# mhamilton723/STEGO

Measured on NVIDIA H100. Metric: train-step images/sec, higher is better.
Workload: dtype bf16

## Files before the change

profiles/attn_bench.py:

```python
import argparse
import os
import sys

import torch

sys.path.insert(0, os.path.dirname(os.path.dirname(os.path.abspath(__file__))))
from stego_b200 import _lib, ops
from _measure import call_ms, card, emit

CHECKS = [(1, 128, 1, 1.5), (2, 785, 6, 1.5), (1, 1601, 12, 1.5), (3, 50, 6, 1.5), (1, 257, 2, 1.5), (1, 3137, 2, 1.0),
          (2, 65, 6, 3.0), (1, 129, 1, 1.0), (1, 256, 3, 1.0), (2, 400, 2, 4.0), (1, 17, 1, 1.0)]


def ref(qkv, B, N, heads):
    E = heads * 64
    q, k, v = qkv.float().view(B, N, 3, heads, 64).permute(2, 0, 3, 1, 4)
    attn = ((q @ k.transpose(-2, -1)) * 0.125).softmax(-1)
    return (attn @ v).transpose(1, 2).reshape(B * N, E)


def rel(a, b):
    return ((a.double() - b.double()).norm() / b.double().norm()).item()


def main():
    ap = argparse.ArgumentParser()
    ap.add_argument("--check-only", action="store_true", help="run the correctness checks only")
    args = ap.parse_args()
    if os.environ.get("STEGO_PROFILE_LIB"):
        _lib.LIB_PATH = os.path.abspath(os.environ["STEGO_PROFILE_LIB"])
    dev = torch.device("cuda:0")
    res = dict(card=card(), check=[])
    torch.manual_seed(3)
    ok = True
    for B, N, heads, scale in CHECKS:
        E = heads * 64
        qkv = (torch.randn(B * N, 3 * E, device=dev) * scale).bfloat16()
        out = torch.full((B * N, E), float("nan"), device=dev, dtype=torch.bfloat16)
        ops.attention(qkv, out, B, N, E, heads)
        torch.cuda.synchronize()
        e = rel(out, ref(qkv, B, N, heads))
        fin = bool(torch.isfinite(out.float()).all())
        res["check"].append(dict(B=B, N=N, heads=heads, scale=scale, rel_l2=e, finite=fin))
        ok &= fin and e < 1e-2
    res["check_ok"] = ok
    if ok and not args.check_only:
        res["time"] = []
        flush = torch.zeros(64 * 1024 * 1024, device=dev)
        for name, B, N, heads in [("c1", 64, 785, 6), ("c2", 64, 1601, 12), ("c3", 32, 3137, 12)]:
            E = heads * 64
            qkv = torch.randn(B * N, 3 * E, device=dev).bfloat16()
            out = torch.empty(B * N, E, device=dev, dtype=torch.bfloat16)
            for _ in range(3):
                ops.attention(qkv, out, B, N, E, heads)
            torch.cuda.synchronize()
            tot = 0.0
            iters = 10
            for _ in range(iters):
                flush.add_(1.0)
                tot += call_ms(lambda: ops.attention(qkv, out, B, N, E, heads))[0]
            ms = tot / iters
            fl = 4.0 * B * heads * N * N * 64
            res["time"].append(dict(config=name, B=B, N=N, heads=heads, us=round(ms * 1e3, 1),
                                    tflops=round(fl / ms / 1e9)))
    emit(res)
    sys.exit(0 if ok else 1)


if __name__ == "__main__":
    main()
```

stego_b200/csrc/attention.cu:

```cuda
#include <stdlib.h>

#include "common.cuh"
#include "host_util.h"

namespace stego {

constexpr int ATT_BQ = 128;
constexpr int ATT_BKV = 64;
constexpr int ATT_D = 64;
constexpr int ATT_STAGES = 4;
constexpr int ATT_THREADS = 288;

constexpr uint32_t ATT_Q_BYTES = 128 * 64 * 2;
constexpr uint32_t ATT_KV_BYTES = 64 * 64 * 2;
constexpr uint32_t ATT_SMEM_Q = 0;
constexpr uint32_t ATT_SMEM_KV = ATT_Q_BYTES;
constexpr uint32_t ATT_SMEM_BAR = ATT_SMEM_KV + ATT_STAGES * 2 * ATT_KV_BYTES;
constexpr uint32_t ATT_SMEM_TOTAL = ATT_SMEM_BAR + 128;

struct AttnParams {
  int N;
  int E;
  float scale_log2e;
};

__global__ void __launch_bounds__(ATT_THREADS, 2)
attention_fwd_kernel(const __grid_constant__ CUtensorMap tmQKV, const __grid_constant__ CUtensorMap tmOut, AttnParams p) {
  extern __shared__ __align__(1024) uint8_t smem[];
  if ((smem_u32(smem) & 1023u) != 0u) __trap();
  uint64_t* bars = reinterpret_cast<uint64_t*>(smem + ATT_SMEM_BAR);
  uint64_t* q_full = bars;
  uint64_t* kv_full = bars + 1;
  uint64_t* kv_empty = kv_full + ATT_STAGES;

  const int warp = threadIdx.x >> 5;
  const int lane = threadIdx.x & 31;
  const int q0 = blockIdx.x * ATT_BQ;
  const int head = blockIdx.y;
  const int img = blockIdx.z;
  const int nkv = (p.N + ATT_BKV - 1) / ATT_BKV;

  if (threadIdx.x == 0) {
    mbar_init(q_full, 1);
    for (int s = 0; s < ATT_STAGES; ++s) {
      mbar_init(&kv_full[s], 1);
      mbar_init(&kv_empty[s], 2);
    }
    fence_barrier_init();
  }
  __syncthreads();

  if (warp == 8) {
    if (lane == 0) {
      tma_prefetch_desc(&tmQKV);
      tma_prefetch_desc(&tmOut);
      mbar_arrive_expect_tx(q_full, ATT_Q_BYTES);
      tma_load_3d(smem + ATT_SMEM_Q, &tmQKV, q_full, head * ATT_D, q0, img);
      tma_load_3d(smem + ATT_SMEM_Q + ATT_Q_BYTES / 2, &tmQKV, q_full, head * ATT_D, q0 + 64, img);
      uint32_t stage = 0, phase = 0;
      for (int j = 0; j < nkv; ++j) {
        mbar_wait(&kv_empty[stage], phase ^ 1u);
        uint8_t* sk = smem + ATT_SMEM_KV + stage * 2 * ATT_KV_BYTES;
        mbar_arrive_expect_tx(&kv_full[stage], 2 * ATT_KV_BYTES);
        tma_load_3d(sk, &tmQKV, &kv_full[stage], p.E + head * ATT_D, j * ATT_BKV, img);
        tma_load_3d(sk + ATT_KV_BYTES, &tmQKV, &kv_full[stage], 2 * p.E + head * ATT_D, j * ATT_BKV, img);
        if (++stage == ATT_STAGES) { stage = 0; phase ^= 1u; }
      }
    }
    return;
  }

  const int wg = warp >> 2;
  const int wq = warp & 3;
  const bool leader = (threadIdx.x & 127) == 0;
  const float c = p.scale_log2e;
  constexpr uint32_t DESC_HI = smem_desc_hi_sw128(1024);
  uint8_t* sq = smem + ATT_SMEM_Q + wg * (ATT_Q_BYTES / 2);
  const uint32_t q_lo = smem_desc_lo(smem_u32(sq), 16);
  const uint32_t k_lo0 = smem_desc_lo(smem_u32(smem + ATT_SMEM_KV), 16);
  const uint32_t v_lo0 = smem_desc_lo(smem_u32(smem + ATT_SMEM_KV + ATT_KV_BYTES), 8192);
  float o[32];
#pragma unroll
  for (int i = 0; i < 32; ++i) o[i] = 0.f;
  float m_run[2] = {-INFINITY, -INFINITY}, l_run[2] = {0.f, 0.f};
  mbar_wait(q_full, 0);
  uint32_t stage = 0, phase = 0;
  for (int j = 0; j < nkv; ++j) {
    mbar_wait(&kv_full[stage], phase);
    const uint32_t k_lo = k_lo0 + stage * ((2 * ATT_KV_BYTES) >> 4);
    const uint32_t v_lo = v_lo0 + stage * ((2 * ATT_KV_BYTES) >> 4);
    float s[32];
    wgmma_fence();
#pragma unroll
    for (uint32_t k = 0; k < ATT_D / 16; ++k)
      wgmma_ss<64, 0, 0>(s, smem_desc_join(q_lo + k * 2, DESC_HI), smem_desc_join(k_lo + k * 2, DESC_HI), k > 0 ? 1u : 0u);
    wgmma_commit();
    wgmma_wait<0>();
    fence_operands(s);
    const int valid = p.N - j * ATT_BKV;
    if (valid < ATT_BKV) {
#pragma unroll
      for (int i = 0; i < 32; ++i)
        if (8 * (i >> 2) + 2 * (lane & 3) + (i & 1) >= valid) s[i] = -INFINITY;
    }
    float alpha[2], mc[2];
#pragma unroll
    for (int h = 0; h < 2; ++h) {
      float mx = -INFINITY;
#pragma unroll
      for (int i = 0; i < 8; ++i) mx = fmaxf(mx, fmaxf(s[4 * i + 2 * h], s[4 * i + 2 * h + 1]));
      mx = fmaxf(mx, __shfl_xor_sync(0xffffffffu, mx, 1));
      mx = fmaxf(mx, __shfl_xor_sync(0xffffffffu, mx, 2));
      const float m_new = fmaxf(m_run[h], mx);
      alpha[h] = ex2_approx((m_run[h] - m_new) * c);
      m_run[h] = m_new;
      mc[h] = m_new * c;
    }
    uint32_t a[4][4];
    float rs[2] = {0.f, 0.f};
#pragma unroll
    for (int i = 0; i < 8; ++i) {
#pragma unroll
      for (int h = 0; h < 2; ++h) {
        const float e0 = ex2_approx(fmaf(s[4 * i + 2 * h], c, -mc[h]));
        const float e1 = ex2_approx(fmaf(s[4 * i + 2 * h + 1], c, -mc[h]));
        rs[h] += e0 + e1;
        a[i >> 1][(i & 1) * 2 + h] = pack_bf16x2(e0, e1);
      }
    }
#pragma unroll
    for (int h = 0; h < 2; ++h) l_run[h] = l_run[h] * alpha[h] + rs[h];
#pragma unroll
    for (int i = 0; i < 32; ++i) o[i] *= alpha[(i >> 1) & 1];
    wgmma_fence();
#pragma unroll
    for (uint32_t kk = 0; kk < ATT_BKV / 16; ++kk)
      wgmma_rs_n64<1>(o, a[kk], smem_desc_join(v_lo + kk * (2048u >> 4), DESC_HI), 1u);
    wgmma_commit();
    wgmma_wait<0>();
    fence_operands(o);
    if (leader) mbar_arrive(&kv_empty[stage]);
    if (++stage == ATT_STAGES) { stage = 0; phase ^= 1u; }
  }
  float inv[2];
#pragma unroll
  for (int h = 0; h < 2; ++h) {
    float l = l_run[h];
    l += __shfl_xor_sync(0xffffffffu, l, 1);
    l += __shfl_xor_sync(0xffffffffu, l, 2);
    inv[h] = __fdividef(1.0f, l);
  }
#pragma unroll
  for (int i = 0; i < 8; ++i) {
#pragma unroll
    for (int h = 0; h < 2; ++h) {
      const uint32_t r = static_cast<uint32_t>(wq * 16 + (lane >> 2) + 8 * h);
      const uint32_t off = sw128_offset(r, static_cast<uint32_t>(i)) + 4u * static_cast<uint32_t>(lane & 3);
      *reinterpret_cast<uint32_t*>(sq + off) = pack_bf16x2(o[4 * i + 2 * h] * inv[h], o[4 * i + 2 * h + 1] * inv[h]);
    }
  }
  fence_proxy_async_smem();
  asm volatile("bar.sync %0, 128;\n" ::"r"(wg + 1) : "memory");
  if (leader) {
    tma_store_3d(sq, &tmOut, head * ATT_D, q0 + wg * 64, img);
    tma_commit_group();
    tma_wait_group_read<0>();
  }
}

constexpr int PRB_STAGES = 4;
constexpr int PRB_PITCH = 72;
constexpr uint32_t PRB_SMEM_K = ATT_Q_BYTES;
constexpr uint32_t PRB_SMEM_STAGE = PRB_SMEM_K + PRB_STAGES * ATT_KV_BYTES;
constexpr uint32_t PRB_WARP_STAGE_BYTES = 16 * PRB_PITCH * 4;
constexpr uint32_t PRB_SMEM_BAR = PRB_SMEM_STAGE + 8 * PRB_WARP_STAGE_BYTES;
constexpr uint32_t PRB_SMEM_TOTAL = PRB_SMEM_BAR + 128;

__device__ __forceinline__ void st_global_cs(float* p, float v) {
  asm volatile("st.global.cs.f32 [%0], %1;\n" ::"l"(p), "f"(v) : "memory");
}

__global__ void __launch_bounds__(ATT_THREADS, 2)
attention_probs_kernel(const __grid_constant__ CUtensorMap tmQKV, float* __restrict__ probs, AttnParams p) {
  extern __shared__ __align__(1024) uint8_t smem[];
  if ((smem_u32(smem) & 1023u) != 0u) __trap();
  uint64_t* bars = reinterpret_cast<uint64_t*>(smem + PRB_SMEM_BAR);
  uint64_t* q_full = bars;
  uint64_t* k_full = bars + 1;
  uint64_t* k_empty = k_full + PRB_STAGES;

  const int warp = threadIdx.x >> 5;
  const int lane = threadIdx.x & 31;
  const int q0 = blockIdx.x * ATT_BQ;
  const int head = blockIdx.y;
  const int img = blockIdx.z;
  const int nkv = (p.N + ATT_BKV - 1) / ATT_BKV;

  if (threadIdx.x == 0) {
    mbar_init(q_full, 1);
    for (int s = 0; s < PRB_STAGES; ++s) {
      mbar_init(&k_full[s], 1);
      mbar_init(&k_empty[s], 2);
    }
    fence_barrier_init();
  }
  __syncthreads();

  if (warp == 8) {
    if (lane == 0) {
      tma_prefetch_desc(&tmQKV);
      mbar_arrive_expect_tx(q_full, ATT_Q_BYTES);
      tma_load_3d(smem, &tmQKV, q_full, head * ATT_D, q0, img);
      tma_load_3d(smem + ATT_Q_BYTES / 2, &tmQKV, q_full, head * ATT_D, q0 + 64, img);
      uint32_t stage = 0, phase = 0;
      for (int j = 0; j < 2 * nkv; ++j) {
        mbar_wait(&k_empty[stage], phase ^ 1u);
        mbar_arrive_expect_tx(&k_full[stage], ATT_KV_BYTES);
        tma_load_3d(smem + PRB_SMEM_K + stage * ATT_KV_BYTES, &tmQKV, &k_full[stage], p.E + head * ATT_D,
                    (j < nkv ? j : j - nkv) * ATT_BKV, img);
        if (++stage == PRB_STAGES) { stage = 0; phase ^= 1u; }
      }
    }
    return;
  }

  const int wg = warp >> 2;
  const int wq = warp & 3;
  const bool leader = (threadIdx.x & 127) == 0;
  const float c = p.scale_log2e;
  constexpr uint32_t DESC_HI = smem_desc_hi_sw128(1024);
  const uint32_t q_lo = smem_desc_lo(smem_u32(smem + wg * (ATT_Q_BYTES / 2)), 16);
  const uint32_t k_lo0 = smem_desc_lo(smem_u32(smem + PRB_SMEM_K), 16);
  float* stage_tile = reinterpret_cast<float*>(smem + PRB_SMEM_STAGE + warp * PRB_WARP_STAGE_BYTES);
  const int row0 = q0 + wg * 64 + wq * 16;
  float m_run[2] = {-INFINITY, -INFINITY}, l_run[2] = {0.f, 0.f};
  float inv[2] = {0.f, 0.f};
  mbar_wait(q_full, 0);
  uint32_t stage = 0, phase = 0;
  for (int j = 0; j < 2 * nkv; ++j) {
    const bool store_pass = j >= nkv;
    const int kt = store_pass ? j - nkv : j;
    mbar_wait(&k_full[stage], phase);
    const uint32_t k_lo = k_lo0 + stage * (ATT_KV_BYTES >> 4);
    float s[32];
    wgmma_fence();
#pragma unroll
    for (uint32_t k = 0; k < ATT_D / 16; ++k)
      wgmma_ss<64, 0, 0>(s, smem_desc_join(q_lo + k * 2, DESC_HI), smem_desc_join(k_lo + k * 2, DESC_HI), k > 0 ? 1u : 0u);
    wgmma_commit();
    wgmma_wait<0>();
    fence_operands(s);
    if (leader) mbar_arrive(&k_empty[stage]);
    if (++stage == PRB_STAGES) { stage = 0; phase ^= 1u; }
    const int valid = p.N - kt * ATT_BKV;
    if (!store_pass) {
      if (valid < ATT_BKV) {
#pragma unroll
        for (int i = 0; i < 32; ++i)
          if (8 * (i >> 2) + 2 * (lane & 3) + (i & 1) >= valid) s[i] = -INFINITY;
      }
#pragma unroll
      for (int h = 0; h < 2; ++h) {
        float mx = -INFINITY;
#pragma unroll
        for (int i = 0; i < 8; ++i) mx = fmaxf(mx, fmaxf(s[4 * i + 2 * h], s[4 * i + 2 * h + 1]));
        mx = fmaxf(mx, __shfl_xor_sync(0xffffffffu, mx, 1));
        mx = fmaxf(mx, __shfl_xor_sync(0xffffffffu, mx, 2));
        const float m_new = fmaxf(m_run[h], mx);
        const float alpha = ex2_approx((m_run[h] - m_new) * c);
        float rs = 0.f;
#pragma unroll
        for (int i = 0; i < 8; ++i)
          rs += ex2_approx((s[4 * i + 2 * h] - m_new) * c) + ex2_approx((s[4 * i + 2 * h + 1] - m_new) * c);
        l_run[h] = l_run[h] * alpha + rs;
        m_run[h] = m_new;
      }
      if (kt == nkv - 1) {
#pragma unroll
        for (int h = 0; h < 2; ++h) {
          float l = l_run[h];
          l += __shfl_xor_sync(0xffffffffu, l, 1);
          l += __shfl_xor_sync(0xffffffffu, l, 2);
          inv[h] = __frcp_rn(l);
        }
      }
      continue;
    }
    __syncwarp();
#pragma unroll
    for (int i = 0; i < 8; ++i) {
#pragma unroll
      for (int h = 0; h < 2; ++h) {
        const float p0 = ex2_approx((s[4 * i + 2 * h] - m_run[h]) * c) * inv[h];
        const float p1 = ex2_approx((s[4 * i + 2 * h + 1] - m_run[h]) * c) * inv[h];
        float2* dst = reinterpret_cast<float2*>(stage_tile + ((lane >> 2) + 8 * h) * PRB_PITCH + 8 * i + 2 * (lane & 3));
        *dst = make_float2(p0, p1);
      }
    }
    __syncwarp();
    const int nrows = min(16, p.N - row0);
    const size_t plane = (static_cast<size_t>(img) * gridDim.y + head) * static_cast<size_t>(p.N);
    float* out = probs + (plane + static_cast<size_t>(row0)) * static_cast<size_t>(p.N) + static_cast<size_t>(kt) * ATT_BKV;
#pragma unroll 4
    for (int r = 0; r < nrows; ++r) {
      float* orow = out + static_cast<size_t>(r) * static_cast<size_t>(p.N);
      if (lane < valid) st_global_cs(orow + lane, stage_tile[r * PRB_PITCH + lane]);
      if (lane + 32 < valid) st_global_cs(orow + lane + 32, stage_tile[r * PRB_PITCH + lane + 32]);
    }
  }
}

}

using namespace stego;

extern "C" int stego_attention_fwd(const void* qkv, void* out, int B, int N, int E, int heads, void* stream_) {
  cudaStream_t stream = reinterpret_cast<cudaStream_t>(stream_);
  STEGO_CHECK_ARG(qkv && out, "stego_attention_fwd: null pointer");
  STEGO_CHECK_ARG(B > 0 && N > 0 && heads > 0, "stego_attention_fwd: bad sizes");
  STEGO_CHECK_ARG(E == heads * ATT_D, "stego_attention_fwd: head_dim must be 64 (E=%d heads=%d)", E, heads);
  STEGO_CHECK_ARG((reinterpret_cast<uintptr_t>(out) & 15u) == 0, "stego_attention_fwd: out not 16-byte aligned");
  CUtensorMap tm;
  uint64_t dims[3] = {(uint64_t)3 * E, (uint64_t)N, (uint64_t)B};
  uint64_t str[2] = {(uint64_t)3 * E * 2, (uint64_t)N * 3 * E * 2};
  uint32_t box[3] = {64, 64, 1};
  int rc = make_tmap_bf16(&tm, qkv, 3, dims, str, box);
  if (rc != STEGO_OK) return rc;
  CUtensorMap tmo;
  uint64_t odims[3] = {(uint64_t)E, (uint64_t)N, (uint64_t)B};
  uint64_t ostr[2] = {(uint64_t)E * 2, (uint64_t)N * E * 2};
  if ((rc = make_tmap_bf16(&tmo, out, 3, odims, ostr, box)) != STEGO_OK) return rc;
  if ((rc = opt_in_smem<attention_fwd_kernel>(ATT_SMEM_TOTAL, "attention_fwd_kernel")) != STEGO_OK) return rc;
  AttnParams p;
  p.N = N;
  p.E = E;
  p.scale_log2e = 0.125f * 1.4426950408889634f;
  dim3 grid((N + ATT_BQ - 1) / ATT_BQ, heads, B);
  attention_fwd_kernel<<<grid, ATT_THREADS, ATT_SMEM_TOTAL, stream>>>(tm, tmo, p);
  STEGO_CHECK_LAUNCH("attention_fwd_kernel");
  return STEGO_OK;
}

extern "C" int stego_attention_probs(const void* qkv, float* probs, int B, int N, int E, int heads, void* stream_) {
  cudaStream_t stream = reinterpret_cast<cudaStream_t>(stream_);
  STEGO_CHECK_ARG(qkv && probs, "stego_attention_probs: null pointer");
  STEGO_CHECK_ARG(B > 0 && N > 0 && heads > 0, "stego_attention_probs: bad sizes");
  STEGO_CHECK_ARG(B <= 65535 && heads <= 65535, "stego_attention_probs: B and heads must be <= 65535");
  STEGO_CHECK_ARG(E == heads * ATT_D, "stego_attention_probs: head_dim must be 64 (E=%d heads=%d)", E, heads);
  STEGO_CHECK_ARG((reinterpret_cast<uintptr_t>(probs) & 3u) == 0, "stego_attention_probs: probs not 4-byte aligned");
  CUtensorMap tm;
  uint64_t dims[3] = {(uint64_t)3 * E, (uint64_t)N, (uint64_t)B};
  uint64_t str[2] = {(uint64_t)3 * E * 2, (uint64_t)N * 3 * E * 2};
  uint32_t box[3] = {64, 64, 1};
  int rc = make_tmap_bf16(&tm, qkv, 3, dims, str, box);
  if (rc != STEGO_OK) return rc;
  if ((rc = opt_in_smem<attention_probs_kernel>(PRB_SMEM_TOTAL, "attention_probs_kernel")) != STEGO_OK) return rc;
  AttnParams p;
  p.N = N;
  p.E = E;
  p.scale_log2e = 0.125f * 1.4426950408889634f;
  dim3 grid((N + ATT_BQ - 1) / ATT_BQ, heads, B);
  attention_probs_kernel<<<grid, ATT_THREADS, PRB_SMEM_TOTAL, stream>>>(tm, probs, p);
  STEGO_CHECK_LAUNCH("attention_probs_kernel");
  return STEGO_OK;
}
```

stego_b200/csrc/common.cuh:

```cuda
#pragma once
#include <cuda.h>
#include <cuda_bf16.h>
#include <cuda_runtime.h>
#include <stdint.h>
#include <stdio.h>

namespace stego {

typedef __nv_bfloat16 bf16;

__device__ __forceinline__ uint32_t smem_u32(const void* p) {
  return static_cast<uint32_t>(__cvta_generic_to_shared(p));
}
__device__ __forceinline__ uint32_t lane_id() { return threadIdx.x & 31u; }

__device__ __forceinline__ float warp_sum(float v) {
#pragma unroll
  for (int o = 16; o > 0; o >>= 1) v += __shfl_xor_sync(0xffffffffu, v, o);
  return v;
}
__device__ __forceinline__ float warp_max(float v) {
#pragma unroll
  for (int o = 16; o > 0; o >>= 1) v = fmaxf(v, __shfl_xor_sync(0xffffffffu, v, o));
  return v;
}

__device__ __forceinline__ void mbar_init(uint64_t* bar, uint32_t count) {
  asm volatile("mbarrier.init.shared::cta.b64 [%0], %1;\n" ::"r"(smem_u32(bar)), "r"(count) : "memory");
}
__device__ __forceinline__ void fence_barrier_init() {
  asm volatile("fence.mbarrier_init.release.cluster;\n" ::: "memory");
}
__device__ __forceinline__ void fence_proxy_async_smem() {
  asm volatile("fence.proxy.async.shared::cta;\n" ::: "memory");
}
__device__ __forceinline__ void mbar_arrive(uint64_t* bar) {
  asm volatile("mbarrier.arrive.shared::cta.b64 _, [%0];\n" ::"r"(smem_u32(bar)) : "memory");
}
__device__ __forceinline__ void mbar_arrive_expect_tx(uint64_t* bar, uint32_t bytes) {
  asm volatile("mbarrier.arrive.expect_tx.shared::cta.b64 _, [%0], %1;\n" ::"r"(smem_u32(bar)), "r"(bytes)
               : "memory");
}
__device__ __forceinline__ bool mbar_try_wait(uint64_t* bar, uint32_t parity) {
  uint32_t ok;
  asm volatile(
      "{\n\t.reg .pred P1;\n\t"
      "mbarrier.try_wait.parity.shared::cta.b64 P1, [%1], %2, %3;\n\t"
      "selp.b32 %0, 1, 0, P1;\n\t}\n"
      : "=r"(ok)
      : "r"(smem_u32(bar)), "r"(parity), "r"(1000000u)
      : "memory");
  return ok != 0;
}

__device__ __forceinline__ bool mbar_test_wait(uint64_t* bar, uint32_t parity) {
  uint32_t ok;
  asm volatile(
      "{\n\t.reg .pred P1;\n\t"
      "mbarrier.test_wait.parity.shared::cta.b64 P1, [%1], %2;\n\t"
      "selp.b32 %0, 1, 0, P1;\n\t}\n"
      : "=r"(ok)
      : "r"(smem_u32(bar)), "r"(parity)
      : "memory");
  return ok != 0;
}

#ifndef STEGO_MBAR_TIMEOUT_NS
#define STEGO_MBAR_TIMEOUT_NS 4000000000ull
#endif
__device__ __forceinline__ uint64_t globaltimer_ns() {
  uint64_t t;
  asm volatile("mov.u64 %0, %%globaltimer;\n" : "=l"(t));
  return t;
}
__device__ __forceinline__ void mbar_wait(uint64_t* bar, uint32_t parity) {
  if (mbar_test_wait(bar, parity)) return;
  if (mbar_try_wait(bar, parity)) return;
  uint32_t spins = 0;
  uint64_t t0 = 0;
  while (!mbar_try_wait(bar, parity)) {
    if ((++spins & 0x3Fu) == 0) {
      const uint64_t now = globaltimer_ns();
      if (t0 == 0) {
        t0 = now;
      } else if (now - t0 > STEGO_MBAR_TIMEOUT_NS) {
        __trap();
      }
    }
  }
}

__device__ __forceinline__ void tma_prefetch_desc(const CUtensorMap* m) {
  asm volatile("prefetch.tensormap [%0];\n" ::"l"(reinterpret_cast<uint64_t>(m)) : "memory");
}
__device__ __forceinline__ void tma_load_2d(void* smem_dst, const CUtensorMap* m, uint64_t* bar, int c0, int c1) {
  asm volatile(
      "cp.async.bulk.tensor.2d.shared::cluster.global.mbarrier::complete_tx::bytes [%0], [%1, {%3, %4}], [%2];\n" ::"r"(
          smem_u32(smem_dst)),
      "l"(reinterpret_cast<uint64_t>(m)), "r"(smem_u32(bar)), "r"(c0), "r"(c1)
      : "memory");
}
__device__ __forceinline__ void tma_load_3d(void* smem_dst, const CUtensorMap* m, uint64_t* bar, int c0, int c1,
                                            int c2) {
  asm volatile(
      "cp.async.bulk.tensor.3d.shared::cluster.global.mbarrier::complete_tx::bytes [%0], [%1, {%3, %4, %5}], "
      "[%2];\n" ::"r"(smem_u32(smem_dst)),
      "l"(reinterpret_cast<uint64_t>(m)), "r"(smem_u32(bar)), "r"(c0), "r"(c1), "r"(c2)
      : "memory");
}

__device__ __forceinline__ void tma_prefetch_l2_2d(const CUtensorMap* m, int c0, int c1) {
  asm volatile("cp.async.bulk.prefetch.tensor.2d.L2.global [%0, {%1, %2}];\n" ::"l"(reinterpret_cast<uint64_t>(m)),
               "r"(c0), "r"(c1)
               : "memory");
}

__device__ __forceinline__ void tma_store_3d(uint32_t smem_src, const CUtensorMap* m, int c0, int c1, int c2) {
  asm volatile("cp.async.bulk.tensor.3d.global.shared::cta.bulk_group [%0, {%2, %3, %4}], [%1];\n" ::"l"(
                   reinterpret_cast<uint64_t>(m)),
               "r"(smem_src), "r"(c0), "r"(c1), "r"(c2)
               : "memory");
}
__device__ __forceinline__ void tma_store_3d(const void* smem_src, const CUtensorMap* m, int c0, int c1, int c2) {
  tma_store_3d(smem_u32(smem_src), m, c0, c1, c2);
}
__device__ __forceinline__ void tma_reduce_add_3d(uint32_t smem_src, const CUtensorMap* m, int c0, int c1, int c2) {
  asm volatile("cp.reduce.async.bulk.tensor.3d.global.shared::cta.add.bulk_group [%0, {%2, %3, %4}], [%1];\n" ::"l"(
                   reinterpret_cast<uint64_t>(m)),
               "r"(smem_src), "r"(c0), "r"(c1), "r"(c2)
               : "memory");
}

__device__ __forceinline__ void st_shared_b32(uint32_t addr, uint32_t v) {
  asm volatile("st.shared.b32 [%0], %1;\n" ::"r"(addr), "r"(v) : "memory");
}
__device__ __forceinline__ void st_shared_v2_f32(uint32_t addr, float a, float b) {
  asm volatile("st.shared.v2.f32 [%0], {%1, %2};\n" ::"r"(addr), "f"(a), "f"(b) : "memory");
}
__device__ __forceinline__ void tma_commit_group() { asm volatile("cp.async.bulk.commit_group;\n" ::: "memory"); }
template <int kPending>
__device__ __forceinline__ void tma_wait_group_read() {
  asm volatile("cp.async.bulk.wait_group.read %0;\n" ::"n"(kPending) : "memory");
}
template <int kPending>
__device__ __forceinline__ void tma_wait_group() {
  asm volatile("cp.async.bulk.wait_group %0;\n" ::"n"(kPending) : "memory");
}

__device__ __forceinline__ void named_bar_sync(int id, int threads) {
  asm volatile("bar.sync %0, %1;\n" ::"r"(id), "r"(threads) : "memory");
}

__device__ __forceinline__ void wgmma_fence() { asm volatile("wgmma.fence.sync.aligned;\n" ::: "memory"); }
__device__ __forceinline__ void wgmma_commit() { asm volatile("wgmma.commit_group.sync.aligned;\n" ::: "memory"); }
template <int kPending>
__device__ __forceinline__ void wgmma_wait() {
  asm volatile("wgmma.wait_group.sync.aligned %0;\n" ::"n"(kPending) : "memory");
}
template <int kN>
__device__ __forceinline__ void fence_operands(float (&d)[kN]) {
#pragma unroll
  for (int i = 0; i < kN; ++i) asm volatile("" : "+f"(d[i])::"memory");
}

template <int kTransA, int kTransB>
__device__ __forceinline__ void wgmma_ss_n64(float (&d)[32], uint64_t desc_a, uint64_t desc_b, uint32_t accumulate) {
  asm volatile(
      "{\n\t.reg .pred p;\n\tsetp.ne.b32 p, %34, 0;\n\t"
      "wgmma.mma_async.sync.aligned.m64n64k16.f32.bf16.bf16 {%0, %1, %2, %3, %4, %5, %6, %7, %8, %9, %10, %11, %12, %13, %14, %15, %16, %17, %18, %19, %20, %21, %22, %23, %24, %25, %26, %27, %28, %29, %30, %31}, %32, %33, p, 1, 1, %35, %36;\n\t}\n"
      : "+f"(d[0]), "+f"(d[1]), "+f"(d[2]), "+f"(d[3]), "+f"(d[4]), "+f"(d[5]), "+f"(d[6]), "+f"(d[7]), "+f"(d[8]), "+f"(d[9]), "+f"(d[10]), "+f"(d[11]), "+f"(d[12]), "+f"(d[13]), "+f"(d[14]), "+f"(d[15]), "+f"(d[16]), "+f"(d[17]), "+f"(d[18]), "+f"(d[19]), "+f"(d[20]), "+f"(d[21]), "+f"(d[22]), "+f"(d[23]), "+f"(d[24]), "+f"(d[25]), "+f"(d[26]), "+f"(d[27]), "+f"(d[28]), "+f"(d[29]), "+f"(d[30]), "+f"(d[31])
      : "l"(desc_a), "l"(desc_b), "r"(accumulate), "n"(kTransA), "n"(kTransB));
}

template <int kTransA, int kTransB>
__device__ __forceinline__ void wgmma_ss_n128(float (&d)[64], uint64_t desc_a, uint64_t desc_b, uint32_t accumulate) {
  asm volatile(
      "{\n\t.reg .pred p;\n\tsetp.ne.b32 p, %66, 0;\n\t"
      "wgmma.mma_async.sync.aligned.m64n128k16.f32.bf16.bf16 {%0, %1, %2, %3, %4, %5, %6, %7, %8, %9, %10, %11, %12, %13, %14, %15, %16, %17, %18, %19, %20, %21, %22, %23, %24, %25, %26, %27, %28, %29, %30, %31, %32, %33, %34, %35, %36, %37, %38, %39, %40, %41, %42, %43, %44, %45, %46, %47, %48, %49, %50, %51, %52, %53, %54, %55, %56, %57, %58, %59, %60, %61, %62, %63}, %64, %65, p, 1, 1, %67, %68;\n\t}\n"
      : "+f"(d[0]), "+f"(d[1]), "+f"(d[2]), "+f"(d[3]), "+f"(d[4]), "+f"(d[5]), "+f"(d[6]), "+f"(d[7]), "+f"(d[8]), "+f"(d[9]), "+f"(d[10]), "+f"(d[11]), "+f"(d[12]), "+f"(d[13]), "+f"(d[14]), "+f"(d[15]), "+f"(d[16]), "+f"(d[17]), "+f"(d[18]), "+f"(d[19]), "+f"(d[20]), "+f"(d[21]), "+f"(d[22]), "+f"(d[23]), "+f"(d[24]), "+f"(d[25]), "+f"(d[26]), "+f"(d[27]), "+f"(d[28]), "+f"(d[29]), "+f"(d[30]), "+f"(d[31]), "+f"(d[32]), "+f"(d[33]), "+f"(d[34]), "+f"(d[35]), "+f"(d[36]), "+f"(d[37]), "+f"(d[38]), "+f"(d[39]), "+f"(d[40]), "+f"(d[41]), "+f"(d[42]), "+f"(d[43]), "+f"(d[44]), "+f"(d[45]), "+f"(d[46]), "+f"(d[47]), "+f"(d[48]), "+f"(d[49]), "+f"(d[50]), "+f"(d[51]), "+f"(d[52]), "+f"(d[53]), "+f"(d[54]), "+f"(d[55]), "+f"(d[56]), "+f"(d[57]), "+f"(d[58]), "+f"(d[59]), "+f"(d[60]), "+f"(d[61]), "+f"(d[62]), "+f"(d[63])
      : "l"(desc_a), "l"(desc_b), "r"(accumulate), "n"(kTransA), "n"(kTransB));
}

template <int kTransA, int kTransB>
__device__ __forceinline__ void wgmma_ss_n256(float (&d)[128], uint64_t desc_a, uint64_t desc_b, uint32_t accumulate) {
  asm volatile(
      "{\n\t.reg .pred p;\n\tsetp.ne.b32 p, %130, 0;\n\t"
      "wgmma.mma_async.sync.aligned.m64n256k16.f32.bf16.bf16 {%0, %1, %2, %3, %4, %5, %6, %7, %8, %9, %10, %11, %12, %13, %14, %15, %16, %17, %18, %19, %20, %21, %22, %23, %24, %25, %26, %27, %28, %29, %30, %31, %32, %33, %34, %35, %36, %37, %38, %39, %40, %41, %42, %43, %44, %45, %46, %47, %48, %49, %50, %51, %52, %53, %54, %55, %56, %57, %58, %59, %60, %61, %62, %63, %64, %65, %66, %67, %68, %69, %70, %71, %72, %73, %74, %75, %76, %77, %78, %79, %80, %81, %82, %83, %84, %85, %86, %87, %88, %89, %90, %91, %92, %93, %94, %95, %96, %97, %98, %99, %100, %101, %102, %103, %104, %105, %106, %107, %108, %109, %110, %111, %112, %113, %114, %115, %116, %117, %118, %119, %120, %121, %122, %123, %124, %125, %126, %127}, %128, %129, p, 1, 1, %131, %132;\n\t}\n"
      : "+f"(d[0]), "+f"(d[1]), "+f"(d[2]), "+f"(d[3]), "+f"(d[4]), "+f"(d[5]), "+f"(d[6]), "+f"(d[7]), "+f"(d[8]), "+f"(d[9]), "+f"(d[10]), "+f"(d[11]), "+f"(d[12]), "+f"(d[13]), "+f"(d[14]), "+f"(d[15]), "+f"(d[16]), "+f"(d[17]), "+f"(d[18]), "+f"(d[19]), "+f"(d[20]), "+f"(d[21]), "+f"(d[22]), "+f"(d[23]), "+f"(d[24]), "+f"(d[25]), "+f"(d[26]), "+f"(d[27]), "+f"(d[28]), "+f"(d[29]), "+f"(d[30]), "+f"(d[31]), "+f"(d[32]), "+f"(d[33]), "+f"(d[34]), "+f"(d[35]), "+f"(d[36]), "+f"(d[37]), "+f"(d[38]), "+f"(d[39]), "+f"(d[40]), "+f"(d[41]), "+f"(d[42]), "+f"(d[43]), "+f"(d[44]), "+f"(d[45]), "+f"(d[46]), "+f"(d[47]), "+f"(d[48]), "+f"(d[49]), "+f"(d[50]), "+f"(d[51]), "+f"(d[52]), "+f"(d[53]), "+f"(d[54]), "+f"(d[55]), "+f"(d[56]), "+f"(d[57]), "+f"(d[58]), "+f"(d[59]), "+f"(d[60]), "+f"(d[61]), "+f"(d[62]), "+f"(d[63]), "+f"(d[64]), "+f"(d[65]), "+f"(d[66]), "+f"(d[67]), "+f"(d[68]), "+f"(d[69]), "+f"(d[70]), "+f"(d[71]), "+f"(d[72]), "+f"(d[73]), "+f"(d[74]), "+f"(d[75]), "+f"(d[76]), "+f"(d[77]), "+f"(d[78]), "+f"(d[79]), "+f"(d[80]), "+f"(d[81]), "+f"(d[82]), "+f"(d[83]), "+f"(d[84]), "+f"(d[85]), "+f"(d[86]), "+f"(d[87]), "+f"(d[88]), "+f"(d[89]), "+f"(d[90]), "+f"(d[91]), "+f"(d[92]), "+f"(d[93]), "+f"(d[94]), "+f"(d[95]), "+f"(d[96]), "+f"(d[97]), "+f"(d[98]), "+f"(d[99]), "+f"(d[100]), "+f"(d[101]), "+f"(d[102]), "+f"(d[103]), "+f"(d[104]), "+f"(d[105]), "+f"(d[106]), "+f"(d[107]), "+f"(d[108]), "+f"(d[109]), "+f"(d[110]), "+f"(d[111]), "+f"(d[112]), "+f"(d[113]), "+f"(d[114]), "+f"(d[115]), "+f"(d[116]), "+f"(d[117]), "+f"(d[118]), "+f"(d[119]), "+f"(d[120]), "+f"(d[121]), "+f"(d[122]), "+f"(d[123]), "+f"(d[124]), "+f"(d[125]), "+f"(d[126]), "+f"(d[127])
      : "l"(desc_a), "l"(desc_b), "r"(accumulate), "n"(kTransA), "n"(kTransB));
}

template <int kTransB>
__device__ __forceinline__ void wgmma_rs_n64(float (&d)[32], const uint32_t (&a)[4], uint64_t desc_b, uint32_t accumulate) {
  asm volatile(
      "{\n\t.reg .pred p;\n\tsetp.ne.b32 p, %37, 0;\n\t"
      "wgmma.mma_async.sync.aligned.m64n64k16.f32.bf16.bf16 {%0, %1, %2, %3, %4, %5, %6, %7, %8, %9, %10, %11, %12, %13, %14, %15, %16, %17, %18, %19, %20, %21, %22, %23, %24, %25, %26, %27, %28, %29, %30, %31}, {%32, %33, %34, %35}, %36, p, 1, 1, %38;\n\t}\n"
      : "+f"(d[0]), "+f"(d[1]), "+f"(d[2]), "+f"(d[3]), "+f"(d[4]), "+f"(d[5]), "+f"(d[6]), "+f"(d[7]), "+f"(d[8]), "+f"(d[9]), "+f"(d[10]), "+f"(d[11]), "+f"(d[12]), "+f"(d[13]), "+f"(d[14]), "+f"(d[15]), "+f"(d[16]), "+f"(d[17]), "+f"(d[18]), "+f"(d[19]), "+f"(d[20]), "+f"(d[21]), "+f"(d[22]), "+f"(d[23]), "+f"(d[24]), "+f"(d[25]), "+f"(d[26]), "+f"(d[27]), "+f"(d[28]), "+f"(d[29]), "+f"(d[30]), "+f"(d[31])
      : "r"(a[0]), "r"(a[1]), "r"(a[2]), "r"(a[3]), "l"(desc_b), "r"(accumulate), "n"(kTransB));
}

template <int N, int kTransA, int kTransB>
__device__ __forceinline__ void wgmma_ss(float (&d)[N / 2], uint64_t desc_a, uint64_t desc_b, uint32_t accumulate) {
  static_assert(N == 64 || N == 128 || N == 256, "wgmma_ss: N must be 64, 128 or 256");
  if constexpr (N == 64) wgmma_ss_n64<kTransA, kTransB>(d, desc_a, desc_b, accumulate);
  else if constexpr (N == 128) wgmma_ss_n128<kTransA, kTransB>(d, desc_a, desc_b, accumulate);
  else wgmma_ss_n256<kTransA, kTransB>(d, desc_a, desc_b, accumulate);
}

template <uint32_t kRegs>
__device__ __forceinline__ void warpgroup_reg_alloc() { asm volatile("setmaxnreg.inc.sync.aligned.u32 %0;\n" ::"n"(kRegs)); }
template <uint32_t kRegs>
__device__ __forceinline__ void warpgroup_reg_dealloc() { asm volatile("setmaxnreg.dec.sync.aligned.u32 %0;\n" ::"n"(kRegs)); }

__device__ __forceinline__ float ex2_approx(float x) {
  float y;
  asm("ex2.approx.ftz.f32 %0, %1;\n" : "=f"(y) : "f"(x));
  return y;
}

__device__ __forceinline__ float ex2_approx_v(float x) {
  float y;
  asm volatile("ex2.approx.ftz.f32 %0, %1;\n" : "=f"(y) : "f"(x));
  return y;
}

__device__ __forceinline__ uint32_t smem_desc_lo(uint32_t smem_addr, uint32_t lbo_bytes) {
  return ((smem_addr & 0x3FFFFu) >> 4) | (((lbo_bytes >> 4) & 0x3FFFu) << 16);
}
__host__ __device__ constexpr uint32_t smem_desc_hi_sw128(uint32_t sbo_bytes) {
  return ((sbo_bytes >> 4) & 0x3FFFu) | (1u << 30);
}
__device__ __forceinline__ uint64_t smem_desc_join(uint32_t lo, uint32_t hi) {
  return (static_cast<uint64_t>(hi) << 32) | lo;
}

__device__ __forceinline__ uint32_t sw128_offset(uint32_t row, uint32_t chunk16) {
  return row * 128u + ((chunk16 ^ (row & 7u)) << 4);
}

__device__ __forceinline__ uint64_t pack_f32x2(float lo, float hi) {
  uint64_t r;
  asm("mov.b64 %0, {%1, %2};\n" : "=l"(r) : "f"(lo), "f"(hi));
  return r;
}
__device__ __forceinline__ void unpack_f32x2(uint64_t v, float& lo, float& hi) {
  asm("mov.b64 {%0, %1}, %2;\n" : "=f"(lo), "=f"(hi) : "l"(v));
}
__device__ __forceinline__ uint64_t fma_f32x2(uint64_t a, uint64_t b, uint64_t c) {
  float a0, a1, b0, b1, c0, c1;
  unpack_f32x2(a, a0, a1); unpack_f32x2(b, b0, b1); unpack_f32x2(c, c0, c1);
  return pack_f32x2(__fmaf_rn(a0, b0, c0), __fmaf_rn(a1, b1, c1));
}
__device__ __forceinline__ uint64_t add_f32x2(uint64_t a, uint64_t b) {
  float a0, a1, b0, b1;
  unpack_f32x2(a, a0, a1); unpack_f32x2(b, b0, b1);
  return pack_f32x2(__fadd_rn(a0, b0), __fadd_rn(a1, b1));
}
__device__ __forceinline__ uint64_t mul_f32x2(uint64_t a, uint64_t b) {
  float a0, a1, b0, b1;
  unpack_f32x2(a, a0, a1); unpack_f32x2(b, b0, b1);
  return pack_f32x2(__fmul_rn(a0, b0), __fmul_rn(a1, b1));
}

__device__ __forceinline__ uint32_t pack_bf16x2(float lo, float hi) {
  __nv_bfloat162 v = __floats2bfloat162_rn(lo, hi);
  return *reinterpret_cast<uint32_t*>(&v);
}

struct AdamCoef {
  float b1, c1, b2, c2;
  float step_size;
  float sqrt_bc2;
  float eps;
};
inline AdamCoef adam_coef(double lr, double beta1, double beta2, double eps, double step) {
  AdamCoef c;
  c.b1 = static_cast<float>(beta1);
  c.c1 = static_cast<float>(1.0 - beta1);
  c.b2 = static_cast<float>(beta2);
  c.c2 = static_cast<float>(1.0 - beta2);
  c.step_size = static_cast<float>(lr / (1.0 - pow(beta1, step)));
  c.sqrt_bc2 = static_cast<float>(sqrt(1.0 - pow(beta2, step)));
  c.eps = static_cast<float>(eps);
  return c;
}
__device__ __forceinline__ void adam_elem(float& p, float& m, float& v, float g, const AdamCoef& c) {
  m = __fmaf_rn(c.c1, g, __fmul_rn(m, c.b1));
  v = __fmaf_rn(__fmul_rn(c.c2, g), g, __fmul_rn(v, c.b2));
  const float denom = __fadd_rn(__fdiv_rn(__fsqrt_rn(v), c.sqrt_bc2), c.eps);
  p = __fmaf_rn(-c.step_size, __fdiv_rn(m, denom), p);
}

}
```

Measured before the change: 3103.

## Narrow last KV tile wgmma and retire idle warpgroup in partial Q blocks

Templates the attention kernel on the width of the final KV tile, so shapes like N=785 (tail 17) run the last QK^T and PV with n16/n32 wgmma instead of a full 64-wide tile. It also lets the second consumer warpgroup exit early when the Q block has at most 64 valid rows, with the kv_empty barrier count adjusted to match. Both aim to cut wasted tensor-core and softmax work on padded rows and columns. The cost is three kernel instantiations and extra code size. The benchmark also gains bit-exact save and compare modes.

```diff
diff --git a/profiles/attn_bench.py b/profiles/attn_bench.py
--- a/profiles/attn_bench.py
+++ b/profiles/attn_bench.py
@@ -23,9 +23,45 @@
     return ((a.double() - b.double()).norm() / b.double().norm()).item()
 
 
+BIT_SHAPES = [("c1", 64, 785, 6), ("c2", 64, 1601, 12), ("c3", 32, 3137, 12)] + \
+    [(f"N{n}", 3, n, 6) for n in (1, 2, 63, 64, 65, 129, 193, 785)]
+
+
+def seeded_outputs(dev):
+    from stego_b200.dino.vision_transformer import vit_small
+    outs = {}
+    for i, (name, B, N, heads) in enumerate(BIT_SHAPES):
+        E = heads * 64
+        for scale in (1.0, 4.0):
+            g = torch.Generator(device=dev).manual_seed(1000 + i)
+            qkv = (torch.randn(B * N, 3 * E, generator=g, device=dev) * scale).bfloat16()
+            out = torch.empty(B * N, E, device=dev, dtype=torch.bfloat16)
+            ops.attention(qkv, out, B, N, E, heads)
+            outs[f"attention_{name}_x{scale:g}"] = out.cpu()
+    torch.manual_seed(0)
+    model = vit_small(patch_size=8).to(dev).eval()
+    img = torch.randn(64, 3, 224, 224, generator=torch.Generator().manual_seed(1)).to(dev)
+    outs["patch_features_c1"] = model.patch_features(img).cpu()
+    return outs
+
+
+def compare_outputs(got, want):
+    res = {}
+    for name, w in want.items():
+        g = got[name]
+        if torch.equal(g.view(torch.int16), w.view(torch.int16)):
+            res[name] = "bit-identical"
+            continue
+        idx = int((g.view(torch.int16) != w.view(torch.int16)).flatten().nonzero()[0])
+        res[name] = dict(first_difference=idx, got=float(g.flatten()[idx]), want=float(w.flatten()[idx]))
+    return res
+
+
 def main():
     ap = argparse.ArgumentParser()
     ap.add_argument("--check-only", action="store_true", help="run the correctness checks only")
+    ap.add_argument("--save-outputs", metavar="PATH", help="save the seeded outputs to PATH instead of timing")
+    ap.add_argument("--compare-outputs", metavar="PATH", help="compare the seeded outputs bit for bit with PATH")
     args = ap.parse_args()
     if os.environ.get("STEGO_PROFILE_LIB"):
         _lib.LIB_PATH = os.path.abspath(os.environ["STEGO_PROFILE_LIB"])
@@ -44,7 +80,15 @@
         res["check"].append(dict(B=B, N=N, heads=heads, scale=scale, rel_l2=e, finite=fin))
         ok &= fin and e < 1e-2
     res["check_ok"] = ok
-    if ok and not args.check_only:
+    if ok and (args.save_outputs or args.compare_outputs):
+        outs = seeded_outputs(dev)
+        if args.save_outputs:
+            torch.save(outs, args.save_outputs)
+            res["saved"] = sorted(outs)
+        else:
+            res["bits"] = compare_outputs(outs, torch.load(args.compare_outputs))
+            ok = all(v == "bit-identical" for v in res["bits"].values())
+    elif ok and not args.check_only:
         res["time"] = []
         flush = torch.zeros(64 * 1024 * 1024, device=dev)
         for name, B, N, heads in [("c1", 64, 785, 6), ("c2", 64, 1601, 12), ("c3", 32, 3137, 12)]:
diff --git a/stego_b200/csrc/attention.cu b/stego_b200/csrc/attention.cu
--- a/stego_b200/csrc/attention.cu
+++ b/stego_b200/csrc/attention.cu
@@ -1,4 +1,6 @@
 #include <stdlib.h>
+
+#include <type_traits>
 
 #include "common.cuh"
 #include "host_util.h"
@@ -24,6 +26,7 @@
   float scale_log2e;
 };
 
+template <int kLastW>
 __global__ void __launch_bounds__(ATT_THREADS, 2)
 attention_fwd_kernel(const __grid_constant__ CUtensorMap tmQKV, const __grid_constant__ CUtensorMap tmOut, AttnParams p) {
   extern __shared__ __align__(1024) uint8_t smem[];
@@ -39,12 +42,13 @@
   const int head = blockIdx.y;
   const int img = blockIdx.z;
   const int nkv = (p.N + ATT_BKV - 1) / ATT_BKV;
+  const bool solo = q0 + 64 >= p.N;
 
   if (threadIdx.x == 0) {
     mbar_init(q_full, 1);
     for (int s = 0; s < ATT_STAGES; ++s) {
       mbar_init(&kv_full[s], 1);
-      mbar_init(&kv_empty[s], 2);
+      mbar_init(&kv_empty[s], solo ? 1 : 2);
     }
     fence_barrier_init();
   }
@@ -71,6 +75,7 @@
   }
 
   const int wg = warp >> 2;
+  if (solo && wg == 1) return;
   const int wq = warp & 3;
   const bool leader = (threadIdx.x & 127) == 0;
   const float c = p.scale_log2e;
@@ -83,24 +88,24 @@
 #pragma unroll
   for (int i = 0; i < 32; ++i) o[i] = 0.f;
   float m_run[2] = {-INFINITY, -INFINITY}, l_run[2] = {0.f, 0.f};
-  mbar_wait(q_full, 0);
   uint32_t stage = 0, phase = 0;
-  for (int j = 0; j < nkv; ++j) {
+  const auto tile = [&](int j, auto width) {
+    constexpr int W = decltype(width)::value;
     mbar_wait(&kv_full[stage], phase);
     const uint32_t k_lo = k_lo0 + stage * ((2 * ATT_KV_BYTES) >> 4);
     const uint32_t v_lo = v_lo0 + stage * ((2 * ATT_KV_BYTES) >> 4);
-    float s[32];
+    float s[W / 2];
     wgmma_fence();
 #pragma unroll
     for (uint32_t k = 0; k < ATT_D / 16; ++k)
-      wgmma_ss<64, 0, 0>(s, smem_desc_join(q_lo + k * 2, DESC_HI), smem_desc_join(k_lo + k * 2, DESC_HI), k > 0 ? 1u : 0u);
+      wgmma_ss<W, 0, 0>(s, smem_desc_join(q_lo + k * 2, DESC_HI), smem_desc_join(k_lo + k * 2, DESC_HI), k > 0 ? 1u : 0u);
     wgmma_commit();
     wgmma_wait<0>();
     fence_operands(s);
     const int valid = p.N - j * ATT_BKV;
-    if (valid < ATT_BKV) {
-#pragma unroll
-      for (int i = 0; i < 32; ++i)
+    if (valid < W) {
+#pragma unroll
+      for (int i = 0; i < W / 2; ++i)
         if (8 * (i >> 2) + 2 * (lane & 3) + (i & 1) >= valid) s[i] = -INFINITY;
     }
     float alpha[2], mc[2];
@@ -108,7 +113,7 @@
     for (int h = 0; h < 2; ++h) {
       float mx = -INFINITY;
 #pragma unroll
-      for (int i = 0; i < 8; ++i) mx = fmaxf(mx, fmaxf(s[4 * i + 2 * h], s[4 * i + 2 * h + 1]));
+      for (int i = 0; i < W / 8; ++i) mx = fmaxf(mx, fmaxf(s[4 * i + 2 * h], s[4 * i + 2 * h + 1]));
       mx = fmaxf(mx, __shfl_xor_sync(0xffffffffu, mx, 1));
       mx = fmaxf(mx, __shfl_xor_sync(0xffffffffu, mx, 2));
       const float m_new = fmaxf(m_run[h], mx);
@@ -116,10 +121,10 @@
       m_run[h] = m_new;
       mc[h] = m_new * c;
     }
-    uint32_t a[4][4];
+    uint32_t a[W / 16][4];
     float rs[2] = {0.f, 0.f};
 #pragma unroll
-    for (int i = 0; i < 8; ++i) {
+    for (int i = 0; i < W / 8; ++i) {
 #pragma unroll
       for (int h = 0; h < 2; ++h) {
         const float e0 = ex2_approx(fmaf(s[4 * i + 2 * h], c, -mc[h]));
@@ -134,14 +139,18 @@
     for (int i = 0; i < 32; ++i) o[i] *= alpha[(i >> 1) & 1];
     wgmma_fence();
 #pragma unroll
-    for (uint32_t kk = 0; kk < ATT_BKV / 16; ++kk)
+    for (uint32_t kk = 0; kk < W / 16; ++kk)
       wgmma_rs_n64<1>(o, a[kk], smem_desc_join(v_lo + kk * (2048u >> 4), DESC_HI), 1u);
     wgmma_commit();
     wgmma_wait<0>();
     fence_operands(o);
     if (leader) mbar_arrive(&kv_empty[stage]);
     if (++stage == ATT_STAGES) { stage = 0; phase ^= 1u; }
-  }
+  };
+  mbar_wait(q_full, 0);
+  const int nfull = kLastW == ATT_BKV ? nkv : nkv - 1;
+  for (int j = 0; j < nfull; ++j) tile(j, std::integral_constant<int, ATT_BKV>{});
+  if constexpr (kLastW < ATT_BKV) tile(nkv - 1, std::integral_constant<int, kLastW>{});
   float inv[2];
 #pragma unroll
   for (int h = 0; h < 2; ++h) {
@@ -314,6 +323,16 @@
 
 using namespace stego;
 
+template <int kLastW>
+static int launch_attention_fwd(const CUtensorMap& tm, const CUtensorMap& tmo, const AttnParams& p, dim3 grid,
+                                cudaStream_t stream) {
+  constexpr auto kern = attention_fwd_kernel<kLastW>;
+  if (const int rc = opt_in_smem<kern>(ATT_SMEM_TOTAL, "attention_fwd_kernel"); rc != STEGO_OK) return rc;
+  kern<<<grid, ATT_THREADS, ATT_SMEM_TOTAL, stream>>>(tm, tmo, p);
+  STEGO_CHECK_LAUNCH("attention_fwd_kernel");
+  return STEGO_OK;
+}
+
 extern "C" int stego_attention_fwd(const void* qkv, void* out, int B, int N, int E, int heads, void* stream_) {
   cudaStream_t stream = reinterpret_cast<cudaStream_t>(stream_);
   STEGO_CHECK_ARG(qkv && out, "stego_attention_fwd: null pointer");
@@ -330,15 +349,16 @@
   uint64_t odims[3] = {(uint64_t)E, (uint64_t)N, (uint64_t)B};
   uint64_t ostr[2] = {(uint64_t)E * 2, (uint64_t)N * E * 2};
   if ((rc = make_tmap_bf16(&tmo, out, 3, odims, ostr, box)) != STEGO_OK) return rc;
-  if ((rc = opt_in_smem<attention_fwd_kernel>(ATT_SMEM_TOTAL, "attention_fwd_kernel")) != STEGO_OK) return rc;
   AttnParams p;
   p.N = N;
   p.E = E;
   p.scale_log2e = 0.125f * 1.4426950408889634f;
   dim3 grid((N + ATT_BQ - 1) / ATT_BQ, heads, B);
-  attention_fwd_kernel<<<grid, ATT_THREADS, ATT_SMEM_TOTAL, stream>>>(tm, tmo, p);
-  STEGO_CHECK_LAUNCH("attention_fwd_kernel");
-  return STEGO_OK;
+  const int tail = N - ((N - 1) / ATT_BKV) * ATT_BKV;
+  if (tail <= 16) rc = launch_attention_fwd<16>(tm, tmo, p, grid, stream);
+  else if (tail <= 32) rc = launch_attention_fwd<32>(tm, tmo, p, grid, stream);
+  else rc = launch_attention_fwd<64>(tm, tmo, p, grid, stream);
+  return rc;
 }
 
 extern "C" int stego_attention_probs(const void* qkv, float* probs, int B, int N, int E, int heads, void* stream_) {
diff --git a/stego_b200/csrc/common.cuh b/stego_b200/csrc/common.cuh
--- a/stego_b200/csrc/common.cuh
+++ b/stego_b200/csrc/common.cuh
@@ -164,6 +164,24 @@
 }
 
 template <int kTransA, int kTransB>
+__device__ __forceinline__ void wgmma_ss_n16(float (&d)[8], uint64_t desc_a, uint64_t desc_b, uint32_t accumulate) {
+  asm volatile(
+      "{\n\t.reg .pred p;\n\tsetp.ne.b32 p, %10, 0;\n\t"
+      "wgmma.mma_async.sync.aligned.m64n16k16.f32.bf16.bf16 {%0, %1, %2, %3, %4, %5, %6, %7}, %8, %9, p, 1, 1, %11, %12;\n\t}\n"
+      : "+f"(d[0]), "+f"(d[1]), "+f"(d[2]), "+f"(d[3]), "+f"(d[4]), "+f"(d[5]), "+f"(d[6]), "+f"(d[7])
+      : "l"(desc_a), "l"(desc_b), "r"(accumulate), "n"(kTransA), "n"(kTransB));
+}
+
+template <int kTransA, int kTransB>
+__device__ __forceinline__ void wgmma_ss_n32(float (&d)[16], uint64_t desc_a, uint64_t desc_b, uint32_t accumulate) {
+  asm volatile(
+      "{\n\t.reg .pred p;\n\tsetp.ne.b32 p, %18, 0;\n\t"
+      "wgmma.mma_async.sync.aligned.m64n32k16.f32.bf16.bf16 {%0, %1, %2, %3, %4, %5, %6, %7, %8, %9, %10, %11, %12, %13, %14, %15}, %16, %17, p, 1, 1, %19, %20;\n\t}\n"
+      : "+f"(d[0]), "+f"(d[1]), "+f"(d[2]), "+f"(d[3]), "+f"(d[4]), "+f"(d[5]), "+f"(d[6]), "+f"(d[7]), "+f"(d[8]), "+f"(d[9]), "+f"(d[10]), "+f"(d[11]), "+f"(d[12]), "+f"(d[13]), "+f"(d[14]), "+f"(d[15])
+      : "l"(desc_a), "l"(desc_b), "r"(accumulate), "n"(kTransA), "n"(kTransB));
+}
+
+template <int kTransA, int kTransB>
 __device__ __forceinline__ void wgmma_ss_n64(float (&d)[32], uint64_t desc_a, uint64_t desc_b, uint32_t accumulate) {
   asm volatile(
       "{\n\t.reg .pred p;\n\tsetp.ne.b32 p, %34, 0;\n\t"
@@ -201,8 +219,10 @@
 
 template <int N, int kTransA, int kTransB>
 __device__ __forceinline__ void wgmma_ss(float (&d)[N / 2], uint64_t desc_a, uint64_t desc_b, uint32_t accumulate) {
-  static_assert(N == 64 || N == 128 || N == 256, "wgmma_ss: N must be 64, 128 or 256");
-  if constexpr (N == 64) wgmma_ss_n64<kTransA, kTransB>(d, desc_a, desc_b, accumulate);
+  static_assert(N == 16 || N == 32 || N == 64 || N == 128 || N == 256, "wgmma_ss: N must be 16, 32, 64, 128 or 256");
+  if constexpr (N == 16) wgmma_ss_n16<kTransA, kTransB>(d, desc_a, desc_b, accumulate);
+  else if constexpr (N == 32) wgmma_ss_n32<kTransA, kTransB>(d, desc_a, desc_b, accumulate);
+  else if constexpr (N == 64) wgmma_ss_n64<kTransA, kTransB>(d, desc_a, desc_b, accumulate);
   else if constexpr (N == 128) wgmma_ss_n128<kTransA, kTransB>(d, desc_a, desc_b, accumulate);
   else wgmma_ss_n256<kTransA, kTransB>(d, desc_a, desc_b, accumulate);
 }
```

After: 3151 (median of 6 runs). 1.5% higher.
